# facebookresearch/habitat-lab

Measured on NVIDIA H100. Metric: DD-PPO learner frames/sec (ResNet18 RGB-D 256x256), higher is better.
Workload: dtype bf16

## Files before the change

### habitat-lab_b200/csrc/conv_halo.cu

```cuda
#include <cuda.h>
#include <stdlib.h>

#include "common.cuh"
#include "wgmma.cuh"

namespace hb200 {
void count_launch(int n);
using namespace wg;

constexpr int TH = 16, TW = 8;

__device__ __forceinline__ float warp_reduce16(float (&v)[16], int lane) {
  float a[8], b[4], c[2];
  const bool b4 = lane & 16, b3 = lane & 8, b2 = lane & 4, b1 = lane & 2;
#pragma unroll
  for (int i = 0; i < 8; ++i) a[i] = (b4 ? v[i + 8] : v[i]) + __shfl_xor_sync(0xffffffffu, b4 ? v[i] : v[i + 8], 16);
#pragma unroll
  for (int i = 0; i < 4; ++i) b[i] = (b3 ? a[i + 4] : a[i]) + __shfl_xor_sync(0xffffffffu, b3 ? a[i] : a[i + 4], 8);
#pragma unroll
  for (int i = 0; i < 2; ++i) c[i] = (b2 ? b[i + 2] : b[i]) + __shfl_xor_sync(0xffffffffu, b2 ? b[i] : b[i + 2], 4);
  float d = (b1 ? c[1] : c[0]) + __shfl_xor_sync(0xffffffffu, b1 ? c[0] : c[1], 2);
  d += __shfl_xor_sync(0xffffffffu, d, 1);
  return d;
}
// ... 340 lines not shown
      mbar_expect_tx(&dy_bar[st], (uint32_t)(DY_BYTES + (XMODE ? HROWS_LOAD * RP : 0)));
      tma_load_4d(sd, tmap_p, &dy_bar[st], 0, ow0, oh0, b);
      if (XMODE == 1) tma_load_5d(sd + DY_BYTES, tmap_xp, &dy_bar[st], 0, ow0 - PAD, 0, oh0 - PAD, b);
      if (XMODE == 2) tma_load_5d(sd + DY_BYTES, tmap_xp, &dy_bar[st], 0, ow0 - PAD, 0, 2 * (oh0 - PAD), b);
    }
  };
  const int first = blockIdx.x, stride = gridDim.x;
  const int my_n = first < a.ntiles ? (a.ntiles - first + stride - 1) / stride : 0;
  if (XMODE == 0 && my_n > 0) {
    fetch_x(first);
    commit_tile(first, 0);
  }
  cp_async_commit();
  fence_proxy_async_smem();
  __syncthreads();
  float acc_w[APC][N];
  auto mma_tile = [&](int it, uint32_t sd) {
    const uint32_t sh = sd + DY_BYTES;
    wgmma_fence();
#pragma unroll
    for (int l = 0; l < APC; ++l) {
      const int ai = grp * APC + l, s = ai / MT, mt = ai % MT;
#pragma unroll
      for (int ks = 0; ks < TH / 2; ++ks) {
        const uint64_t da = make_smem_desc(sh + 2 * ks * RP + s * 16 + mt * 16 * P, RP, P, kNoSwizzle);
        const uint64_t db = make_smem_desc(sd + ks * (16 * N * 2), 0, 8 * N * 2, N == 64 ? kSwizzle128B : kSwizzle64B);
        mma128<N, kBF16, 1, 1>(acc_w[l], da, 8 * P, db, (it > 0 || ks > 0) ? 1u : 0u);
      }
    }
    wgmma_commit();
    wgmma_wait<0>();
  };

  if (XMODE != 0) {
    if (tid == 0)
      for (int p = 0; p < NSW - 1 && p < my_n; ++p) commit_tile(first + p * stride, p);
    for (int it = 0; it < my_n; ++it) {
      const int nxt = it + NSW - 1;
      if (tid == 0 && nxt < my_n) commit_tile(first + nxt * stride, nxt % NSW);
      mbar_wait(&dy_bar[it % NSW], (it / NSW) & 1);
      mma_tile(it, sbase + (it % NSW) * STAGE);
    }
  } else {
    for (int it = 0; it < my_n; ++it) {
      const bool more = it + 1 < my_n;
      if (more) fetch_x(first + (it + 1) * stride);
      if (more) commit_tile(first + (it + 1) * stride, (it + 1) & 1);
      cp_async_commit();
      cp_async_wait<1>();
      fence_proxy_async_smem();
      __syncthreads();
      mbar_wait(&dy_bar[it & 1], (it >> 1) & 1);
      mma_tile(it, sbase + (it & 1) * STAGE);
    }
  }
  {
#pragma unroll
    for (int l = 0; l < APC; ++l) {
      if (my_n == 0) {
#pragma unroll
        for (int j = 0; j < N; ++j) acc_w[l][j] = 0.f;
      }
      acc_fence(acc_w[l]);
      const int ai = grp * APC + l, s = ai / MT, mt = ai % MT;
      const int blk = mt * 16 + (tid >> 3);
      const int r = blk / CJ, cj = blk % CJ;
      const bool ok = r < KH;
      const size_t row = (size_t)(r * KW + s) * C + cj * 8 + (tid & 7);
#pragma unroll
      for (int col0 = 0; col0 < N; col0 += 32) {
        float rr[32];
        acc_row32(acc_w[l], col0, stage_buf, rr);
        if (ok) {
          float* dst = a.dw + ((size_t)blockIdx.x * (KH * KW * C) + row) * N + col0;
#pragma unroll
          for (int j = 0; j < 32; j += 4) *reinterpret_cast<float4*>(dst + j) = make_float4(rr[j], rr[j + 1], rr[j + 2], rr[j + 3]);
        }
      }
    }
  }
}


constexpr int kSmallWgradStages = 3;
struct HaloWgradSmallArgs {
  const grad_t* x;
  const grad_t* dy;
  float* dw;
  int B, Ci, Co, ntiles;
};

template <int NS, int IMG>
__global__ void __launch_bounds__(128)
conv_halo_wgrad_small_kernel(const HaloWgradSmallArgs a, const __grid_constant__ CUtensorMap tmap_dy) {
  constexpr int CJ = 4, KH = 3, KW = 3, HWD = TW + KW - 1;
  constexpr int P = HWD * 16, RP = CJ * P;
  constexpr int IPT = TH / IMG;
  constexpr int RPI = IMG + 2;
  constexpr int HROWS_LOAD = IPT * RPI;
  constexpr int HROWS = (IPT - 1) * RPI + (IMG - 2) + 1 + 4;
  constexpr int HROWS_A = HROWS > HROWS_LOAD ? HROWS : HROWS_LOAD;
  constexpr int HALO_BYTES = (HROWS_A * RP + 1023) / 1024 * 1024;
  constexpr int NB = NS / 64;
  constexpr int DY_BYTES = NB * 128 * 128;
  constexpr int STAGE = HALO_BYTES + DY_BYTES;
  constexpr int NST = kSmallWgradStages;
  static_assert(NS <= 128, "one 128 x NS accumulator per CTA");
  extern __shared__ __align__(16) uint8_t smem_raw[];
  __shared__ __align__(8) uint64_t dy_bar[NST];
  __shared__ float stage_buf[kStageFloats];
  const uint32_t sbase = (smem_u32(smem_raw) + 1023u) & ~1023u;
  const int tid = threadIdx.x, warp = tid >> 5;
  const int nsl = a.Co / NS;
  const int s_tap = blockIdx.y % KW, slice = blockIdx.y / KW;
  const int c_off = (slice / nsl) * 32, n_off = (slice % nsl) * NS;
  const CUtensorMap* const tmap_p = &tmap_dy;

  if (tid == 0) {
#pragma unroll
    for (int i = 0; i < NST; ++i) mbar_init(&dy_bar[i], 1);
    mbar_fence_init();
  }
  for (int st = 0; st < NST; ++st)
    for (int v = tid; v < (HROWS_A - HROWS_LOAD) * RP / 16; v += 128) {
      const uint32_t addr = sbase + st * STAGE + HROWS_LOAD * RP + v * 16;
      asm volatile("st.shared.v4.b32 [%0], {%1,%1,%1,%1};" ::"r"(addr), "r"(0u) : "memory");
    }
  constexpr int XV = HROWS_LOAD * CJ * HWD, XPER = (XV + 95) / 96;
  uint4 xr[XPER];
  auto fetch_x = [&](int tile) {
    if (warp == 0) return;
    const int lt = tid - 32;
    const int b0 = tile * IPT;
#pragma unroll
    for (int i = 0; i < XPER; ++i) {
      const int v = lt + i * 96;
      uint4 r = make_uint4(0u, 0u, 0u, 0u);
      if (v < XV) {
        const int cj = v % CJ;
        const int t = v / CJ;
        const int hx = t % HWD, hy = t / HWD;
        const int j = hy / RPI, ih = hy - j * RPI - 1, iw = hx - 1;
        const int b = b0 + j;
        if (b < a.B && ih >= 0 && ih < IMG && iw >= 0 && iw < IMG)
          r = __ldg(reinterpret_cast<const uint4*>(a.x + ((((size_t)b * IMG + ih) * IMG + iw) * a.Ci + c_off + cj * 8)));
      }
      xr[i] = r;
    }
  };
  auto store_x = [&](int st) {
    if (warp == 0) return;
    const int lt = tid - 32;
    const uint32_t sh = sbase + st * STAGE;
#pragma unroll
    for (int i = 0; i < XPER; ++i) {
      const int v = lt + i * 96;
      if (v < XV) {
        const int cj = v % CJ;
        const int t = v / CJ;
        const int hx = t % HWD, hy = t / HWD;
        asm volatile("st.shared.v4.b32 [%0], {%1,%2,%3,%4};" ::"r"(sh + (uint32_t)(((hy * CJ + cj) * HWD + hx) * 16)),
                     "r"(xr[i].x), "r"(xr[i].y), "r"(xr[i].z), "r"(xr[i].w) : "memory");
      }
    }
  };
  auto load_dy = [&, tmap_p](int tile, int st) {
    const uint32_t sd = sbase + st * STAGE + HALO_BYTES;
    mbar_expect_tx(&dy_bar[st], (uint32_t)DY_BYTES);
#pragma unroll
    for (int nb = 0; nb < NB; ++nb)
      tma_load_4d(sd + (uint32_t)nb * (128 * 128), tmap_p, &dy_bar[st], n_off + nb * 64, 0, 0, tile * IPT);
  };
  const int first = blockIdx.x, stride = gridDim.x;
  const int my_n = first < a.ntiles ? (a.ntiles - first + stride - 1) / stride : 0;
#pragma unroll
  for (int i = 0; i < NST - 1; ++i) {
    if (i < my_n) {
      fetch_x(first + i * stride);
      store_x(i);
      if (tid == 0) load_dy(first + i * stride, i);
    }
  }
  fence_proxy_async_smem();
  __syncthreads();
  float acc_t[NS];

  for (int it = 0; it < my_n; ++it) {
    const int st = it % NST;
    const int nt = it + NST - 1;
    if (nt < my_n) fetch_x(first + nt * stride);
    fence_proxy_async_smem();
    __syncthreads();
    mbar_wait(&dy_bar[st], (it / NST) & 1);
    {
      const uint32_t sh = sbase + st * STAGE;
      const uint32_t sd = sh + HALO_BYTES;
      wgmma_fence();
#pragma unroll
      for (int ks = 0; ks < TH / 2; ++ks) {
        const int hb = ((2 * ks) / IMG) * RPI + (2 * ks) % IMG;
        const uint64_t da = make_smem_desc(sh + hb * RP + s_tap * 16, RP, P, kNoSwizzle);
        const uint64_t db = make_smem_desc(sd + ks * 2048, 128 * 128, 1024, kSwizzle128B);
        mma128<NS, kBF16, 1, 1>(acc_t, da, 8 * P, db, (it > 0 || ks > 0) ? 1u : 0u);
      }
      wgmma_commit();
      wgmma_wait<0>();
    }
    if (nt < my_n) {
      store_x(nt % NST);
      if (tid == 0) load_dy(first + nt * stride, nt % NST);
    }
  }
  {
    if (my_n == 0) {
#pragma unroll
      for (int j = 0; j < NS; ++j) acc_t[j] = 0.f;
    }
    acc_fence(acc_t);
    const int blk = tid >> 3;
    const int r = blk / CJ, cj = blk % CJ;
    const bool ok = r < KH;
    const size_t row = (size_t)(r * KW + s_tap) * a.Ci + c_off + cj * 8 + (tid & 7);
#pragma unroll
    for (int col0 = 0; col0 < NS; col0 += 32) {
      float rr[32];
      acc_row32(acc_t, col0, stage_buf, rr);
      if (ok) {
        float* dst = a.dw + ((size_t)blockIdx.x * 9 * a.Ci + row) * a.Co + n_off + col0;
#pragma unroll
        for (int j = 0; j < 32; j += 4) *reinterpret_cast<float4*>(dst + j) = make_float4(rr[j], rr[j + 1], rr[j + 2], rr[j + 3]);
      }
    }
  }
}

__global__ void pack_halo_weight_kernel(const float* __restrict__ w, __nv_bfloat16* __restrict__ img, int KH,
                                        int KW, int C, int N, int co, int ci_real, int mode) {
  const long long total = (long long)KH * KW * C * N;
  for (long long i = blockIdx.x * (long long)blockDim.x + threadIdx.x; i < total;
       i += (long long)gridDim.x * blockDim.x) {
    const int e = (int)(i & 7);
    long long t = i >> 3;
    const int n = (int)(t % N);
    t /= N;
    const int cj = (int)(t % (C / 8));
    const int tap = (int)(t / (C / 8));
    const int r = tap / KW, s = tap % KW, k = cj * 8 + e;
    float v = 0.f;
    if (mode == 0) {
      if (k < ci_real) v = w[(((size_t)n * ci_real + k) * KH + r) * KW + s];
    } else if (mode == 1) {
      if (n < ci_real) v = w[(((size_t)k * ci_real + n) * KH + (KH - 1 - r)) * KW + (KW - 1 - s)];
    } else {
      const int dy = k >> 3, dx = (k >> 2) & 1, c = k & 3;
      const int fr = 2 * r + dy - 1, fs = 2 * s + dx - 1;
      if (c < ci_real && fr >= 0 && fr < 7 && fs >= 0 && fs < 7) v = w[(((size_t)n * ci_real + c) * 7 + fr) * 7 + fs];
    }
    if (mode == 1) img[i] = __float2bfloat16(v);
    else reinterpret_cast<__half*>(img)[i] = __float2half_rn(v);
  }
}

__global__ void unpack_stem_wgrad_kernel(const float* __restrict__ acc, float* __restrict__ dw, int co, int ci_real) {
  const int total = co * ci_real * 49;
  for (int i = blockIdx.x * blockDim.x + threadIdx.x; i < total; i += gridDim.x * blockDim.x) {
    const int fs = i % 7, fr = (i / 7) % 7, c = (i / 49) % ci_real, o = i / (49 * ci_real);
    const int a = (fr + 1) >> 1, dy = (fr + 1) & 1, b = (fs + 1) >> 1, dx = (fs + 1) & 1;
    dw[i] = acc[((size_t)(a * 4 + b) * 16 + (dy * 2 + dx) * 4 + c) * co + o];
  }
}


template <int C, int N, int KH, int KW, int PAD, int MODE>
__global__ void __launch_bounds__(128)
conv_halo_tma_kernel(const HaloArgs a, const __grid_constant__ CUtensorMap tmap) {
  using Cfg = HaloCfg<C, N, KH, KW, PAD>;
  constexpr int CJ = Cfg::CJ, HH = Cfg::HH, HWD = Cfg::HWD;
  constexpr uint32_t SLAB = (uint32_t)((HH * HWD * 16 + 127) / 128 * 128);
  constexpr uint32_t STAGE = CJ * SLAB;
  constexpr int NB = (Cfg::W_BYTES + 2 * (int)STAGE > 110 * 1024) ? 1 : 2;
  extern __shared__ __align__(16) uint8_t smem_raw[];
  __shared__ __align__(8) uint64_t ld_bar[2];
  __shared__ float stage_buf[kStageFloats];
  const uint32_t sbase = (smem_u32(smem_raw) + 127u) & ~127u;
  const uint32_t s_w = sbase;
  const uint32_t s_halo0 = s_w + Cfg::W_BYTES;
  const int tid = threadIdx.x, lane = tid & 31;

  if (tid == 0) {
    mbar_init(&ld_bar[0], 1);
    mbar_init(&ld_bar[1], 1);
    mbar_fence_init();
  }
  {
    const uint4* src = reinterpret_cast<const uint4*>(a.wimg);
    for (int v = tid; v < Cfg::W_BYTES / 16; v += 128) cp_async16(s_w + (uint32_t)v * 16, src + v, true);
  }
  cp_async_commit();
  const int tiles_x = a.W / TW, tiles_y = a.H / TH;
  const int tiles_per_img = tiles_x * tiles_y;
  auto tile_coords = [&](int tile, int& b, int& oh0, int& ow0) {
    b = tile / tiles_per_img;
    const int r = tile - b * tiles_per_img;
    oh0 = (r / tiles_x) * TH;
    ow0 = (r % tiles_x) * TW;
  };
  const CUtensorMap* const tmap_p = &tmap;
  auto issue_halo = [&, tmap_p](int tile, int stage) {
    int b, oh0, ow0;
    tile_coords(tile, b, oh0, ow0);
    mbar_expect_tx(&ld_bar[stage], (uint32_t)(CJ * HH * HWD * 16));
#pragma unroll
    for (int j = 0; j < CJ; ++j)
// ... 269 lines not shown
    const int py = t >> 3, px = t & 7;
    float* const stage_buf = stage_bufs + wgi * kStageFloats;
    float acc_t[N];
    for (int it = wgi; it < my_n; it += 2) {
      const int st = it % NS;
      const int tile = first + it * stride;
      const int b = tile / tiles_per_img, r = tile - b * tiles_per_img;
      const int oh0 = (r / tiles_x) * TH, ow0 = (r % tiles_x) * TW;
      mbar_wait(&full_bar[st], (it / NS) & 1);
      const uint32_t sh = s_halo0 + (uint32_t)st * STAGE;
      wgmma_fence();
      uint32_t accum = 0;
#pragma unroll
      for (int r = 0; r < KH; ++r)
#pragma unroll
        for (int s = 0; s < KW; ++s)
#pragma unroll
          for (int kk = 0; kk < C / 16; ++kk) {
            const uint64_t da = SW ? make_smem_desc(sh + s * COPY + r * ATOM + kk * 32, 16, ATOM, (Layout)kSw)
                                   : make_smem_desc(sh + 2 * kk * SLAB + r * (HWD * 16) + s * 16, SLAB, HWD * 16, kNoSwizzle);
            const uint64_t db = make_smem_desc(s_w + (r * KW + s) * (C * N * 2) + 2 * kk * (N * 16), N * 16, 128, kNoSwizzle);
            mma128<N, kT>(acc_t, da, SW ? 8 * ATOM : 8 * HWD * 16, db, accum);
            accum = 1;
          }
      wgmma_commit();
      wgmma_wait<0>();
      acc_fence(acc_t);
      if (t == 0) mbar_arrive(&empty_bar[st]);
      const size_t pix = ((size_t)b * a.H + oh0 + py) * a.W + ow0 + px;
#pragma unroll
      for (int col0 = 0; col0 < N; col0 += 32) {
        float acc_[32];
        acc_row32(acc_t, col0, stage_buf, acc_, 1 + wgi);
        if (MODE == 0 && a.stats != nullptr)
          halo_gn_stats_chunk(acc_, lane, N / a.gn_groups, a.stats + (size_t)b * a.gn_groups * 2, col0);
        const size_t o = pix * N + col0;
        if (MODE == 1 && a.addend != nullptr) {
          const uint4* ad = reinterpret_cast<const uint4*>(a.addend + o);
#pragma unroll
          for (int v = 0; v < 4; ++v) {
            float f[8];
            unpack8(ad[v], f);
#pragma unroll
            for (int e2 = 0; e2 < 8; ++e2) acc_[v * 8 + e2] += f[e2];
          }
        }
        uint4* dst = reinterpret_cast<uint4*>(a.y + o);
#pragma unroll
        for (int v = 0; v < 4; ++v) {
          uint4 u;
          if (MODE == 0) {
            u.x = pack_f16x2(acc_[v * 8 + 0], acc_[v * 8 + 1]);
            u.y = pack_f16x2(acc_[v * 8 + 2], acc_[v * 8 + 3]);
            u.z = pack_f16x2(acc_[v * 8 + 4], acc_[v * 8 + 5]);
            u.w = pack_f16x2(acc_[v * 8 + 6], acc_[v * 8 + 7]);
          } else {
            u.x = pack_bf16x2(acc_[v * 8 + 0], acc_[v * 8 + 1]);
            u.y = pack_bf16x2(acc_[v * 8 + 2], acc_[v * 8 + 3]);
            u.z = pack_bf16x2(acc_[v * 8 + 4], acc_[v * 8 + 5]);
            u.w = pack_bf16x2(acc_[v * 8 + 6], acc_[v * 8 + 7]);
          }
          dst[v] = u;
        }
      }
    }
  }
}

typedef CUresult (*EncodeTiledFn)(CUtensorMap*, CUtensorMapDataType, cuuint32_t, void*, const cuuint64_t*,
                                  const cuuint64_t*, const cuuint32_t*, const cuuint32_t*, CUtensorMapInterleave,
                                  CUtensorMapSwizzle, CUtensorMapL2promotion, CUtensorMapFloatOOBfill);
static EncodeTiledFn halo_encode_fn() {
  static EncodeTiledFn fn = nullptr;
  if (fn) return fn;
  void* p = nullptr;
  cudaDriverEntryPointQueryResult q;
  if (cudaGetDriverEntryPoint("cuTensorMapEncodeTiled", &p, cudaEnableDefault, &q) != cudaSuccess ||
      q != cudaDriverEntryPointSuccess)
    return nullptr;
  fn = (EncodeTiledFn)p;
  return fn;
}

static int blocks_per_sm(const void* kern, size_t smem, int* cache) {
  if (*cache > 0) return *cache;
  cudaFuncAttributes fa;
  if (cudaFuncGetAttributes(&fa, kern) != cudaSuccess) return 1;
  const int regs = fa.numRegs > 0 ? fa.numRegs : 128;
  int by_regs = 65536 / (((regs + 7) / 8 * 8) * 128);
  int by_smem = (int)((227 * 1024) / (smem + fa.sharedSizeBytes + 1024));
  int n = by_regs < by_smem ? by_regs : by_smem;
  if (n > 16) n = 16;
  if (n < 1) n = 1;
  *cache = n;
  return n;
}

template <int C, int N, int KH, int KW, int PAD, int MODE>
static int launch_halo(const HaloArgs& a, cudaStream_t st) {
  using Cfg = HaloCfg<C, N, KH, KW, PAD>;
  const size_t smem = Cfg::W_BYTES + Cfg::NBUF * Cfg::HALO_BYTES + 256;
  auto kern = conv_halo_kernel<C, N, KH, KW, PAD, MODE>;
  static int cache = 0;
  if (cache == 0) HB_CUDA(cudaFuncSetAttribute(kern, cudaFuncAttributeMaxDynamicSharedMemorySize, (int)smem));
  const int per_sm = blocks_per_sm((const void*)kern, smem, &cache);
  int grid = kNumSMs * per_sm;
  if (grid > a.ntiles) grid = a.ntiles;
  kern<<<grid, 128, smem, st>>>(a);
  HB_LAUNCH_OK();
  count_launch(1);
  return HB200_OK;
}

template <int C, int N, int KH, int KW, int PAD, int MODE>
static int launch_halo_tma(const HaloArgs& a, cudaStream_t st) {
  using Cfg = HaloCfg<C, N, KH, KW, PAD>;
  EncodeTiledFn enc = halo_encode_fn();
  if (!enc) {
    set_last_error("conv_halo (TMA): cuTensorMapEncodeTiled is not available from this driver");
    return HB200_ERR_UNSUPPORTED;
  }
  CUtensorMap tmap;
  const cuuint64_t dims[4] = {(cuuint64_t)C, (cuuint64_t)a.W, (cuuint64_t)a.H, (cuuint64_t)a.B};
  const cuuint64_t strides[3] = {(cuuint64_t)C * 2, (cuuint64_t)a.W * C * 2, (cuuint64_t)a.H * a.W * C * 2};
  const cuuint32_t box[4] = {8u, (cuuint32_t)Cfg::HWD, (cuuint32_t)Cfg::HH, 1u};
  const cuuint32_t estr[4] = {1u, 1u, 1u, 1u};
  const CUresult r = enc(&tmap, CU_TENSOR_MAP_DATA_TYPE_BFLOAT16, 4, (void*)a.x, dims, strides, box, estr,
                         CU_TENSOR_MAP_INTERLEAVE_NONE, CU_TENSOR_MAP_SWIZZLE_NONE, CU_TENSOR_MAP_L2_PROMOTION_L2_128B,
                         CU_TENSOR_MAP_FLOAT_OOB_FILL_NONE);
  if (r != CUDA_SUCCESS) {
    set_last_error("conv_halo (TMA): cuTensorMapEncodeTiled failed (%d)", (int)r);
    return HB200_ERR_CUDA;
  }
  constexpr size_t slab = (size_t)((Cfg::HH * Cfg::HWD * 16 + 127) / 128 * 128);
  constexpr int nstage = (Cfg::W_BYTES + 2 * (int)(Cfg::CJ * slab) > 110 * 1024) ? 1 : 2;
  const size_t smem = Cfg::W_BYTES + nstage * Cfg::CJ * slab + 256;
  auto kern = conv_halo_tma_kernel<C, N, KH, KW, PAD, MODE>;
  static int cache = 0;
  if (cache == 0) HB_CUDA(cudaFuncSetAttribute(kern, cudaFuncAttributeMaxDynamicSharedMemorySize, (int)smem));
  const int per_sm = blocks_per_sm((const void*)kern, smem, &cache);
  int grid = kNumSMs * per_sm;
  if (grid > a.ntiles) grid = a.ntiles;
  kern<<<grid, 128, smem, st>>>(a, tmap);
  HB_LAUNCH_OK();
  count_launch(1);
  return HB200_OK;
}

template <int C, int N, int KH, int KW, int PAD, int MODE, int NS, bool SW = false>
static int launch_halo_ws(const HaloArgs& a, cudaStream_t st) {
  using Cfg = HaloCfg<C, N, KH, KW, PAD>;
  EncodeTiledFn enc = halo_encode_fn();
  if (!enc) {
    set_last_error("conv_halo (TMA): cuTensorMapEncodeTiled is not available from this driver");
    return HB200_ERR_UNSUPPORTED;
  }
  CUtensorMap tmap;
  const cuuint64_t dims[4] = {(cuuint64_t)C, (cuuint64_t)a.W, (cuuint64_t)a.H, (cuuint64_t)a.B};
  const cuuint64_t strides[3] = {(cuuint64_t)C * 2, (cuuint64_t)a.W * C * 2, (cuuint64_t)a.H * a.W * C * 2};
  const cuuint32_t box_slab[4] = {8u, (cuuint32_t)Cfg::HWD, (cuuint32_t)Cfg::HH, 1u};
  const cuuint32_t box_rows[4] = {(cuuint32_t)C, (cuuint32_t)TW, (cuuint32_t)Cfg::HH, 1u};
  const cuuint32_t* box = SW ? box_rows : box_slab;
  const cuuint32_t estr[4] = {1u, 1u, 1u, 1u};
  const CUresult r = enc(&tmap, CU_TENSOR_MAP_DATA_TYPE_BFLOAT16, 4, (void*)a.x, dims, strides, box, estr,
                         CU_TENSOR_MAP_INTERLEAVE_NONE,
                         !SW ? CU_TENSOR_MAP_SWIZZLE_NONE : (C == 64 ? CU_TENSOR_MAP_SWIZZLE_128B : CU_TENSOR_MAP_SWIZZLE_64B),
                         CU_TENSOR_MAP_L2_PROMOTION_L2_128B, CU_TENSOR_MAP_FLOAT_OOB_FILL_NONE);
  if (r != CUDA_SUCCESS) {
    set_last_error("conv_halo (TMA): cuTensorMapEncodeTiled failed (%d)", (int)r);
    return HB200_ERR_CUDA;
  }
  constexpr size_t slab = (size_t)((Cfg::HH * Cfg::HWD * 16 + 127) / 128 * 128);
// ... 37 lines not shown
                         CU_TENSOR_MAP_L2_PROMOTION_L2_128B, CU_TENSOR_MAP_FLOAT_OOB_FILL_NONE);
  if (r != CUDA_SUCCESS) {
    set_last_error("conv_halo (swizzled TMA): cuTensorMapEncodeTiled failed (%d)", (int)r);
    return HB200_ERR_CUDA;
  }
  constexpr size_t stage = (size_t)3 * Cfg::HH * 8 * C * 2;
  constexpr int nstage = (Cfg::W_BYTES + 2 * (int)stage > 200 * 1024) ? 1 : 2;
  const size_t smem = Cfg::W_BYTES + nstage * stage + 1024;
  auto kern = conv_halo_sw_kernel<C, N, MODE>;
  static int cache = 0;
  if (cache == 0) HB_CUDA(cudaFuncSetAttribute(kern, cudaFuncAttributeMaxDynamicSharedMemorySize, (int)smem));
  const int per_sm = blocks_per_sm((const void*)kern, smem, &cache);
  int grid = kNumSMs * per_sm;
  if (grid > a.ntiles) grid = a.ntiles;
  kern<<<grid, 128, smem, st>>>(a, tmap);
  HB_LAUNCH_OK();
  count_launch(1);
  return HB200_OK;
}

template <int C, int N, int KH, int KW, int PAD, int XMODE = 0>
static int launch_halo_wgrad(const HaloWgradArgs& a, cudaStream_t st) {
  constexpr int CJ = C / 8, HWD = TW + KW - 1, P = HWD * 16, RP = CJ * P;
  constexpr int MT = (KH * CJ + 15) / 16, RMAX = (MT * 16 + CJ - 1) / CJ, HROWS = TH - 1 + RMAX;
  constexpr int STAGE = (128 * N * 2 + HROWS * RP + 1023) / 1024 * 1024;
  constexpr int NSW = halo_wgrad_stages(XMODE, C, STAGE);
  const size_t smem = NSW * (size_t)STAGE + 1024 + 64;
  EncodeTiledFn enc = halo_encode_fn();
  if (!enc) {
    set_last_error("conv_halo_wgrad: cuTensorMapEncodeTiled is not available from this driver");
    return HB200_ERR_UNSUPPORTED;
  }
  CUtensorMap tmap;
  const cuuint64_t dims[4] = {(cuuint64_t)N, (cuuint64_t)a.W, (cuuint64_t)a.H, (cuuint64_t)a.B};
  const cuuint64_t strides[3] = {(cuuint64_t)N * 2, (cuuint64_t)a.W * N * 2, (cuuint64_t)a.H * a.W * N * 2};
  const cuuint32_t box[4] = {(cuuint32_t)N, (cuuint32_t)TW, (cuuint32_t)TH, 1u};
  const cuuint32_t estr[4] = {1u, 1u, 1u, 1u};
  const CUresult r = enc(&tmap, CU_TENSOR_MAP_DATA_TYPE_BFLOAT16, 4, (void*)a.dy, dims, strides, box, estr,
                         CU_TENSOR_MAP_INTERLEAVE_NONE, N == 64 ? CU_TENSOR_MAP_SWIZZLE_128B : CU_TENSOR_MAP_SWIZZLE_64B,
                         CU_TENSOR_MAP_L2_PROMOTION_L2_128B, CU_TENSOR_MAP_FLOAT_OOB_FILL_NONE);
  if (r != CUDA_SUCCESS) {
    set_last_error("conv_halo_wgrad: cuTensorMapEncodeTiled failed (%d)", (int)r);
    return HB200_ERR_CUDA;
  }
  CUtensorMap tmap_x = tmap;
  if (XMODE != 0) {
    const int cx = XMODE == 2 ? C / 4 : C, hx = XMODE == 2 ? 2 * a.H : a.H, wx = XMODE == 2 ? 2 * a.W : a.W;
    const int chunks_per_row = XMODE == 2 ? CJ / 2 : CJ, col_bytes = (XMODE == 2 ? 2 : 1) * cx * 2;
    const cuuint64_t xd[5] = {8u, (cuuint64_t)a.W, (cuuint64_t)chunks_per_row, (cuuint64_t)hx, (cuuint64_t)a.B};
    const cuuint64_t xs[4] = {(cuuint64_t)col_bytes, 16u, (cuuint64_t)wx * cx * 2, (cuuint64_t)hx * wx * cx * 2};
    constexpr int HROWS_LOAD = TH + KH - 1;
    const cuuint32_t xb[5] = {8u, (cuuint32_t)HWD, (cuuint32_t)chunks_per_row,
                              (cuuint32_t)(XMODE == 2 ? 2 * HROWS_LOAD : HROWS_LOAD), 1u};
    const cuuint32_t xe[5] = {1u, 1u, 1u, 1u, 1u};
    const CUresult rx = enc(&tmap_x, CU_TENSOR_MAP_DATA_TYPE_BFLOAT16, 5, (void*)a.x, xd, xs, xb, xe,
                            CU_TENSOR_MAP_INTERLEAVE_NONE, CU_TENSOR_MAP_SWIZZLE_NONE, CU_TENSOR_MAP_L2_PROMOTION_L2_128B,
                            CU_TENSOR_MAP_FLOAT_OOB_FILL_NONE);
    if (rx != CUDA_SUCCESS) {
      set_last_error("conv_halo_wgrad: cuTensorMapEncodeTiled (x halo) failed (%d)", (int)rx);
      return HB200_ERR_CUDA;
    }
  }
  auto kern = conv_halo_wgrad_kernel<C, N, KH, KW, PAD, XMODE>;
  static int cache = 0;
  if (cache == 0) HB_CUDA(cudaFuncSetAttribute(kern, cudaFuncAttributeMaxDynamicSharedMemorySize, (int)smem));
  constexpr int nacc = KW * MT, ngrp = nacc * N <= 128 ? 1 : nacc / (128 / N);
  const int per_sm = blocks_per_sm((const void*)kern, smem, &cache);
  int grid = kNumSMs * per_sm / ngrp;
  if (grid < 1) grid = 1;
  if (grid > a.ntiles) grid = a.ntiles;
  const long long count = (long long)KH * KW * C * N;
  float* parts = nullptr;
  int* tickets = nullptr;
  int rc = stream_workspace(st, (size_t)(grid + (grid < kReduceChunks ? grid : kReduceChunks)) * count, 0, &parts, &tickets);
  if (rc) return rc;
  HaloWgradArgs ap = a;
  ap.dw = parts;
  kern<<<dim3(grid, ngrp), 128, smem, st>>>(ap, tmap, tmap_x);
  HB_LAUNCH_OK();
  count_launch(1);
  return reduce_partials(parts, grid, count, count, a.dw, parts + (size_t)grid * count, st);
}

template <int NS, int IMG>
static int launch_halo_wgrad_small(const HaloWgradSmallArgs& a, cudaStream_t st) {
  constexpr int RP = 4 * (TW + 2) * 16, IPT = TH / IMG, RPI = IMG + 2;
  constexpr int HROWS_LOAD = IPT * RPI, HROWS = (IPT - 1) * RPI + (IMG - 2) + 1 + 4;
  constexpr int HROWS_A = HROWS > HROWS_LOAD ? HROWS : HROWS_LOAD;
  constexpr int HALO_BYTES = (HROWS_A * RP + 1023) / 1024 * 1024;
  const size_t smem = kSmallWgradStages * (size_t)(HALO_BYTES + (NS / 64) * 128 * 128) + 1024 + 64;
  EncodeTiledFn enc = halo_encode_fn();
  if (!enc) {
    set_last_error("conv_halo_wgrad (small images): cuTensorMapEncodeTiled is not available from this driver");
    return HB200_ERR_UNSUPPORTED;
  }
  CUtensorMap tmap;
  const cuuint64_t dims[4] = {(cuuint64_t)a.Co, (cuuint64_t)IMG, (cuuint64_t)IMG, (cuuint64_t)a.B};
  const cuuint64_t strides[3] = {(cuuint64_t)a.Co * 2, (cuuint64_t)IMG * a.Co * 2, (cuuint64_t)IMG * IMG * a.Co * 2};
  const cuuint32_t box[4] = {64u, 8u, (cuuint32_t)IMG, (cuuint32_t)IPT};
  const cuuint32_t estr[4] = {1u, 1u, 1u, 1u};
  const CUresult r = enc(&tmap, CU_TENSOR_MAP_DATA_TYPE_BFLOAT16, 4, (void*)a.dy, dims, strides, box, estr,
                         CU_TENSOR_MAP_INTERLEAVE_NONE, CU_TENSOR_MAP_SWIZZLE_128B, CU_TENSOR_MAP_L2_PROMOTION_L2_128B,
                         CU_TENSOR_MAP_FLOAT_OOB_FILL_NONE);
  if (r != CUDA_SUCCESS) {
    set_last_error("conv_halo_wgrad (small images): cuTensorMapEncodeTiled failed (%d)", (int)r);
    return HB200_ERR_CUDA;
  }
  auto kern = conv_halo_wgrad_small_kernel<NS, IMG>;
  static bool attr = false;
  if (!attr) {
    HB_CUDA(cudaFuncSetAttribute(kern, cudaFuncAttributeMaxDynamicSharedMemorySize, (int)smem));
    attr = true;
  }
  const int slices = (a.Ci / 32) * (a.Co / NS) * 3;
  int workers = 2 * kNumSMs / slices;
  if (workers < 1) workers = 1;
  if (workers > a.ntiles) workers = a.ntiles;
  const long long count = 9LL * a.Ci * a.Co;
  float* parts = nullptr;
  int* tickets = nullptr;
  int rc = stream_workspace(st, (size_t)(workers + (workers < kReduceChunks ? workers : kReduceChunks)) * count, 0, &parts,
                            &tickets);
  if (rc) return rc;
  HaloWgradSmallArgs ap = a;
  ap.dw = parts;
  kern<<<dim3(workers, slices), 128, smem, st>>>(ap, tmap);
  HB_LAUNCH_OK();
  count_launch(1);
  return reduce_partials(parts, workers, count, count, a.dw, parts + (size_t)workers * count, st);
}
}

using namespace hb200;

static int g_halo_tma = getenv("HB200_NO_HALO_TMA") == nullptr ? 1 : 0;
static int g_wgrad_xtma = getenv("HB200_WGRAD_XTMA") ? atoi(getenv("HB200_WGRAD_XTMA")) : 1;
extern "C" int hb200_set_halo_tma(int enable) {
  g_halo_tma = enable;
  return HB200_OK;
}
extern "C" int hb200_get_halo_tma(void) { return g_halo_tma; }

extern "C" int hb200_conv_halo_supported(int c, int n, int k, int h, int w) {
  if (h % TH || w % TW) return 0;
  if (k == 3) return (c == 32 && n == 32) || (c == 64 && n == 64);
  if (k == 4) return c == 16 && n == 32;
  return 0;
}

extern "C" int hb200_conv_halo_wgrad_supported(int c, int n, int k, int h, int w) {
  if (hb200_conv_halo_supported(c, n, k, h, w)) return 1;
  return k == 3 && c % 32 == 0 && n % 128 == 0 && h == w && (h == 8 || h == 4);
}

extern "C" int hb200_pack_halo_weight(const float* w_oihw, hb200_bf16* img, int co, int ci_real, int c, int n,
                                      int k, int mode, hb200_stream_t stream) {
  HB_CHECK_ARG(w_oihw && img && mode >= 0 && mode <= 2, "pack_halo_weight: bad args");
  const long long total = (long long)k * k * c * n;
  pack_halo_weight_kernel<<<(int)min((total + 255) / 256, (long long)kNumSMs * 4), 256, 0, (cudaStream_t)stream>>>(
      w_oihw, (__nv_bfloat16*)img, k, k, c, n, co, ci_real, mode);
  HB_LAUNCH_OK();
  count_launch(1);
  return HB200_OK;
}

extern "C" int hb200_unpack_stem_wgrad(const float* dw_acc, float* dw_oihw, int co, int ci_real,
                                       hb200_stream_t stream) {
  HB_CHECK_ARG(dw_acc && dw_oihw && ci_real <= 4, "unpack_stem_wgrad: bad args");
  unpack_stem_wgrad_kernel<<<cdiv(co * ci_real * 49, 256), 256, 0, (cudaStream_t)stream>>>(dw_acc, dw_oihw, co, ci_real);
  HB_LAUNCH_OK();
  count_launch(1);
  return HB200_OK;
}

extern "C" int hb200_conv_halo(const hb200_bf16* x, const hb200_bf16* wimg, hb200_bf16* y, const hb200_bf16* addend,
                               double* gn_stats, int gn_groups, int batch, int h, int w, int c, int n, int k,
                               int mode, hb200_stream_t stream) {
  HB_CHECK_ARG(x && wimg && y, "conv_halo: null pointer");
  HB_CHECK_ARG(hb200_conv_halo_supported(c, n, k, h, w), "conv_halo: unsupported shape C=%d N=%d k=%d %dx%d", c, n, k, h, w);
  if (gn_stats) HB_CHECK_ARG(gn_groups > 0 && n % gn_groups == 0 && n / gn_groups >= 2, "conv_halo: bad GroupNorm groups");
  HaloArgs a;
  a.x = (const __nv_bfloat16*)x; a.wimg = (const __nv_bfloat16*)wimg; a.y = (__nv_bfloat16*)y;
  a.addend = (const __nv_bfloat16*)addend; a.stats = gn_stats;
  a.B = batch; a.H = h; a.W = w; a.gn_groups = gn_groups > 0 ? gn_groups : 1;
  a.ntiles = batch * (h / TH) * (w / TW);
  cudaStream_t st = (cudaStream_t)stream;
  const bool use_tma = g_halo_tma != 0;
  if (g_halo_tma == 1 && k == 3 && c == 64)
    return mode == 0 ? launch_halo_ws<64, 64, 3, 3, 1, 0, 2, true>(a, st) : launch_halo_ws<64, 64, 3, 3, 1, 1, 2, true>(a, st);
  if (g_halo_tma == 1 && k == 3 && c == 32)
    return mode == 0 ? launch_halo_ws<32, 32, 3, 3, 1, 0, 6, true>(a, st) : launch_halo_ws<32, 32, 3, 3, 1, 1, 6, true>(a, st);
  if (g_halo_tma == 1 && k == 4 && mode == 0) return launch_halo_ws<16, 32, 4, 4, 2, 0, 6>(a, st);
  if (g_halo_tma == 6 && k == 3 && c == 32)
    return mode == 0 ? launch_halo_ws<32, 32, 3, 3, 1, 0, 2, true>(a, st) : launch_halo_ws<32, 32, 3, 3, 1, 1, 2, true>(a, st);
  if (g_halo_tma == 4 && k == 3 && c == 32)
    return mode == 0 ? launch_halo_ws<32, 32, 3, 3, 1, 0, 3, true>(a, st) : launch_halo_ws<32, 32, 3, 3, 1, 1, 3, true>(a, st);
  if (g_halo_tma == 4 && k == 3 && c == 64)
    return mode == 0 ? launch_halo_ws<64, 64, 3, 3, 1, 0, 2, true>(a, st) : launch_halo_ws<64, 64, 3, 3, 1, 1, 2, true>(a, st);
  if (g_halo_tma == 3 && k == 3 && c == 32)
    return mode == 0 ? launch_halo_ws<32, 32, 3, 3, 1, 0, 4>(a, st) : launch_halo_ws<32, 32, 3, 3, 1, 1, 4>(a, st);
  if (g_halo_tma == 3 && k == 3 && c == 64)
    return mode == 0 ? launch_halo_ws<64, 64, 3, 3, 1, 0, 5>(a, st) : launch_halo_ws<64, 64, 3, 3, 1, 1, 5>(a, st);
  if (g_halo_tma == 3 && k == 4 && mode == 0) return launch_halo_ws<16, 32, 4, 4, 2, 0, 6>(a, st);
  if (g_halo_tma == 2 && k == 3 && c == 32)
    return mode == 0 ? launch_halo_sw<32, 32, 0>(a, st) : launch_halo_sw<32, 32, 1>(a, st);
  if (g_halo_tma == 2 && k == 3 && c == 64)
    return mode == 0 ? launch_halo_sw<64, 64, 0>(a, st) : launch_halo_sw<64, 64, 1>(a, st);
  if (use_tma && k == 3 && c == 32)
    return mode == 0 ? launch_halo_tma<32, 32, 3, 3, 1, 0>(a, st) : launch_halo_tma<32, 32, 3, 3, 1, 1>(a, st);
  if (use_tma && k == 4 && mode == 0) return launch_halo_tma<16, 32, 4, 4, 2, 0>(a, st);
  if (use_tma && k == 3 && c == 64)
    return mode == 0 ? launch_halo_tma<64, 64, 3, 3, 1, 0>(a, st) : launch_halo_tma<64, 64, 3, 3, 1, 1>(a, st);
  if (k == 3 && c == 32) return mode == 0 ? launch_halo<32, 32, 3, 3, 1, 0>(a, st) : launch_halo<32, 32, 3, 3, 1, 1>(a, st);
  if (k == 3 && c == 64) return mode == 0 ? launch_halo<64, 64, 3, 3, 1, 0>(a, st) : launch_halo<64, 64, 3, 3, 1, 1>(a, st);
  HB_CHECK_ARG(mode == 0, "conv_halo: the stem has no data gradient");
  return launch_halo<16, 32, 4, 4, 2, 0>(a, st);
}

__global__ void unpack_s2_wgrad_kernel(const float* __restrict__ acc, float* __restrict__ dw, int co, int ci) {
  const int total = co * ci * 9;
  for (int i = blockIdx.x * blockDim.x + threadIdx.x; i < total; i += gridDim.x * blockDim.x) {
    const int s = i % 3, r = (i / 3) % 3, c = (i / 9) % ci, o = i / (9 * ci);
    const int ky = r == 0 ? 0 : 1, dy = r == 0 ? 1 : r - 1, kx = s == 0 ? 0 : 1, dx = s == 0 ? 1 : s - 1;
    dw[i] = acc[((size_t)((ky * 2 + kx) * 4 + dy * 2 + dx) * ci + c) * co + o];
  }
}

extern "C" int hb200_conv_s2_wgrad_supported(int c, int n, int h, int w) {
  return c == 32 && n == 64 && h % (2 * TH) == 0 && w % (2 * TW) == 0;
}
extern "C" int hb200_conv_s2_wgrad(const hb200_bf16* x, const hb200_bf16* dy, float* dw_acc, int batch, int h, int w,
                                   int c, int n, hb200_stream_t stream) {
  HB_CHECK_ARG(x && dy && dw_acc && batch > 0, "conv_s2_wgrad: null pointer");
  HB_CHECK_ARG(hb200_conv_s2_wgrad_supported(c, n, h, w), "conv_s2_wgrad: unsupported shape C=%d N=%d %dx%d", c, n, h, w);
  HaloWgradArgs a;
  a.x = (const __nv_bfloat16*)x; a.dy = (const __nv_bfloat16*)dy; a.dw = dw_acc;
  a.B = batch; a.H = h / 2; a.W = w / 2;
  a.ntiles = batch * (a.H / TH) * (a.W / TW);
  return launch_halo_wgrad<128, 64, 2, 2, 1, 2>(a, (cudaStream_t)stream);
}
extern "C" int hb200_unpack_s2_wgrad(const float* dw_acc, float* dw_oihw, int co, int ci, hb200_stream_t stream) {
  HB_CHECK_ARG(dw_acc && dw_oihw && co > 0 && ci > 0, "unpack_s2_wgrad: bad args");
  unpack_s2_wgrad_kernel<<<cdiv(co * ci * 9, 256), 256, 0, (cudaStream_t)stream>>>(dw_acc, dw_oihw, co, ci);
  HB_LAUNCH_OK();
  count_launch(1);
  return HB200_OK;
}

extern "C" int hb200_conv_halo_wgrad(const hb200_bf16* x, const hb200_bf16* dy, float* dw_acc, int batch, int h,
                                     int w, int c, int n, int k, hb200_stream_t stream) {
  HB_CHECK_ARG(x && dy && dw_acc, "conv_halo_wgrad: null pointer");
  HB_CHECK_ARG(hb200_conv_halo_wgrad_supported(c, n, k, h, w), "conv_halo_wgrad: unsupported shape C=%d N=%d k=%d %dx%d", c, n, k, h, w);
  if (!hb200_conv_halo_supported(c, n, k, h, w)) {
    HaloWgradSmallArgs s;
    s.x = (const grad_t*)x; s.dy = (const grad_t*)dy; s.dw = dw_acc;
    s.B = batch; s.Ci = c; s.Co = n;
    const int ipt = TH / h;
    s.ntiles = (batch + ipt - 1) / ipt;
    return h == 8 ? launch_halo_wgrad_small<128, 8>(s, (cudaStream_t)stream) : launch_halo_wgrad_small<128, 4>(s, (cudaStream_t)stream);
  }
  HaloWgradArgs a;
  a.x = (const __nv_bfloat16*)x; a.dy = (const __nv_bfloat16*)dy; a.dw = dw_acc;
  a.B = batch; a.H = h; a.W = w;
  a.ntiles = batch * (h / TH) * (w / TW);
  cudaStream_t st = (cudaStream_t)stream;
  if (g_wgrad_xtma) {
    if (k == 3 && c == 32) return launch_halo_wgrad<32, 32, 3, 3, 1, 1>(a, st);
    if (k == 3 && c == 64) return launch_halo_wgrad<64, 64, 3, 3, 1, 1>(a, st);
    return launch_halo_wgrad<16, 32, 4, 4, 2, 1>(a, st);
  }
  if (k == 3 && c == 32) return launch_halo_wgrad<32, 32, 3, 3, 1>(a, st);
  if (k == 3 && c == 64) return launch_halo_wgrad<64, 64, 3, 3, 1>(a, st);
  return launch_halo_wgrad<16, 32, 4, 4, 2>(a, st);
}
extern "C" int hb200_set_wgrad_xtma(int on) { g_wgrad_xtma = on ? 1 : 0; return HB200_OK; }
extern "C" int hb200_get_wgrad_xtma(void) { return g_wgrad_xtma; }
```

Before: 57400.

## Warp-specialize small-image halo wgrad with TMA producer and deep mbarrier pipeline

Replaces the 128-thread small-image weight-gradient kernel with a 416-thread warp-specialized kernel. One producer warpgroup loads both dy and the x halo through TMA (a new 5D tensor map), feeding up to 8 stages guarded by full/empty mbarriers. Three consumer warpgroups each handle one kernel row and use 64-channel input blocks. This removes register-staged x loads and per-iteration __syncthreads, and keeps one wgmma group in flight. The grid is now sized from measured occupancy. The cost is large shared memory per CTA and fewer CTAs per SM.

New measurement: 59880, median of 6. 1.04x the previous value.

```diff
diff --git a/habitat-lab_b200/csrc/conv_halo.cu b/habitat-lab_b200/csrc/conv_halo.cu
--- a/habitat-lab_b200/csrc/conv_halo.cu
+++ b/habitat-lab_b200/csrc/conv_halo.cu
@@ -446,153 +446,109 @@
 }
 
 
-constexpr int kSmallWgradStages = 3;
-struct HaloWgradSmallArgs {
-  const grad_t* x;
-  const grad_t* dy;
+constexpr int kWgradSmallThreads = 416;
+constexpr int kWgradSmallCols = 128;
+struct WgradSmallArgs {
   float* dw;
-  int B, Ci, Co, ntiles;
+  int Ci, Co, ntiles;
 };
 
-template <int NS, int IMG>
-__global__ void __launch_bounds__(128)
-conv_halo_wgrad_small_kernel(const HaloWgradSmallArgs a, const __grid_constant__ CUtensorMap tmap_dy) {
-  constexpr int CJ = 4, KH = 3, KW = 3, HWD = TW + KW - 1;
-  constexpr int P = HWD * 16, RP = CJ * P;
-  constexpr int IPT = TH / IMG;
-  constexpr int RPI = IMG + 2;
-  constexpr int HROWS_LOAD = IPT * RPI;
-  constexpr int HROWS = (IPT - 1) * RPI + (IMG - 2) + 1 + 4;
-  constexpr int HROWS_A = HROWS > HROWS_LOAD ? HROWS : HROWS_LOAD;
-  constexpr int HALO_BYTES = (HROWS_A * RP + 1023) / 1024 * 1024;
-  constexpr int NB = NS / 64;
-  constexpr int DY_BYTES = NB * 128 * 128;
-  constexpr int STAGE = HALO_BYTES + DY_BYTES;
-  constexpr int NST = kSmallWgradStages;
-  static_assert(NS <= 128, "one 128 x NS accumulator per CTA");
+template <int IMG>
+struct WgradSmallCfg {
+  static constexpr int NIMG = TH / IMG;
+  static constexpr int ROWB = IMG * 16;
+  static constexpr int CHUNK = NIMG * (IMG + 2) * ROWB;
+  static constexpr int XB = 8 * CHUNK;
+  static constexpr int DYBLK = TH * TW * 128;
+  static constexpr int DYB = kWgradSmallCols / 64 * DYBLK;
+  static constexpr int GAP = 1024;
+  static constexpr int STAGE = DYB + XB + GAP;
+  static constexpr int NS_FIT = (227 * 1024 - 1024 - 256) / STAGE;
+  static constexpr int NS = NS_FIT < 8 ? NS_FIT : 8;
+  static constexpr size_t SMEM = (size_t)NS * STAGE + 1024;
+  static_assert(XB % 1024 == 0 && NS >= 3, "stage layout");
+};
+
+template <int IMG>
+__global__ void __launch_bounds__(kWgradSmallThreads, 1)
+conv_wgrad_small_ws_kernel(const WgradSmallArgs a, const __grid_constant__ CUtensorMap tmap_dy,
+                           const __grid_constant__ CUtensorMap tmap_x) {
+  using Cfg = WgradSmallCfg<IMG>;
+  constexpr int NS = Cfg::NS, STAGE = Cfg::STAGE, NCO = kWgradSmallCols;
   extern __shared__ __align__(16) uint8_t smem_raw[];
-  __shared__ __align__(8) uint64_t dy_bar[NST];
-  __shared__ float stage_buf[kStageFloats];
+  __shared__ __align__(8) uint64_t full_bar[NS], empty_bar[NS];
   const uint32_t sbase = (smem_u32(smem_raw) + 1023u) & ~1023u;
-  const int tid = threadIdx.x, warp = tid >> 5;
-  const int nsl = a.Co / NS;
-  const int s_tap = blockIdx.y % KW, slice = blockIdx.y / KW;
-  const int c_off = (slice / nsl) * 32, n_off = (slice % nsl) * NS;
-  const CUtensorMap* const tmap_p = &tmap_dy;
-
+  const int tid = threadIdx.x, wg_id = tid >> 7, t = tid & 127;
+  const int nci = (a.Ci + 63) / 64;
+  const int s_tap = blockIdx.y % 3, cb = (blockIdx.y / 3) % nci, nb = blockIdx.y / (3 * nci);
   if (tid == 0) {
 #pragma unroll
-    for (int i = 0; i < NST; ++i) mbar_init(&dy_bar[i], 1);
+    for (int i = 0; i < NS; ++i) {
+      mbar_init(&full_bar[i], 1);
+      mbar_init(&empty_bar[i], 3);
+    }
     mbar_fence_init();
   }
-  for (int st = 0; st < NST; ++st)
-    for (int v = tid; v < (HROWS_A - HROWS_LOAD) * RP / 16; v += 128) {
-      const uint32_t addr = sbase + st * STAGE + HROWS_LOAD * RP + v * 16;
-      asm volatile("st.shared.v4.b32 [%0], {%1,%1,%1,%1};" ::"r"(addr), "r"(0u) : "memory");
-    }
-  constexpr int XV = HROWS_LOAD * CJ * HWD, XPER = (XV + 95) / 96;
-  uint4 xr[XPER];
-  auto fetch_x = [&](int tile) {
-    if (warp == 0) return;
-    const int lt = tid - 32;
-    const int b0 = tile * IPT;
-#pragma unroll
-    for (int i = 0; i < XPER; ++i) {
-      const int v = lt + i * 96;
-      uint4 r = make_uint4(0u, 0u, 0u, 0u);
-      if (v < XV) {
-        const int cj = v % CJ;
-        const int t = v / CJ;
-        const int hx = t % HWD, hy = t / HWD;
-        const int j = hy / RPI, ih = hy - j * RPI - 1, iw = hx - 1;
-        const int b = b0 + j;
-        if (b < a.B && ih >= 0 && ih < IMG && iw >= 0 && iw < IMG)
-          r = __ldg(reinterpret_cast<const uint4*>(a.x + ((((size_t)b * IMG + ih) * IMG + iw) * a.Ci + c_off + cj * 8)));
-      }
-      xr[i] = r;
-    }
-  };
-  auto store_x = [&](int st) {
-    if (warp == 0) return;
-    const int lt = tid - 32;
-    const uint32_t sh = sbase + st * STAGE;
-#pragma unroll
-    for (int i = 0; i < XPER; ++i) {
-      const int v = lt + i * 96;
-      if (v < XV) {
-        const int cj = v % CJ;
-        const int t = v / CJ;
-        const int hx = t % HWD, hy = t / HWD;
-        asm volatile("st.shared.v4.b32 [%0], {%1,%2,%3,%4};" ::"r"(sh + (uint32_t)(((hy * CJ + cj) * HWD + hx) * 16)),
-                     "r"(xr[i].x), "r"(xr[i].y), "r"(xr[i].z), "r"(xr[i].w) : "memory");
-      }
-    }
-  };
-  auto load_dy = [&, tmap_p](int tile, int st) {
-    const uint32_t sd = sbase + st * STAGE + HALO_BYTES;
-    mbar_expect_tx(&dy_bar[st], (uint32_t)DY_BYTES);
-#pragma unroll
-    for (int nb = 0; nb < NB; ++nb)
-      tma_load_4d(sd + (uint32_t)nb * (128 * 128), tmap_p, &dy_bar[st], n_off + nb * 64, 0, 0, tile * IPT);
-  };
+  if (tid < NS * 8)
+    asm volatile("st.shared.v4.b32 [%0], {%1,%1,%1,%1};" ::"r"(sbase + (tid / 8) * STAGE + Cfg::DYB + Cfg::XB + (tid % 8) * 16),
+                 "r"(0u) : "memory");
+  fence_proxy_async_smem();
+  __syncthreads();
   const int first = blockIdx.x, stride = gridDim.x;
   const int my_n = first < a.ntiles ? (a.ntiles - first + stride - 1) / stride : 0;
-#pragma unroll
-  for (int i = 0; i < NST - 1; ++i) {
-    if (i < my_n) {
-      fetch_x(first + i * stride);
-      store_x(i);
-      if (tid == 0) load_dy(first + i * stride, i);
-    }
-  }
-  fence_proxy_async_smem();
-  __syncthreads();
-  float acc_t[NS];
-
-  for (int it = 0; it < my_n; ++it) {
-    const int st = it % NST;
-    const int nt = it + NST - 1;
-    if (nt < my_n) fetch_x(first + nt * stride);
-    fence_proxy_async_smem();
-    __syncthreads();
-    mbar_wait(&dy_bar[st], (it / NST) & 1);
-    {
-      const uint32_t sh = sbase + st * STAGE;
-      const uint32_t sd = sh + HALO_BYTES;
+
+  if (wg_id == 3) {
+    if (t == 0) {
+      const CUtensorMap* const pd = &tmap_dy;
+      const CUtensorMap* const px = &tmap_x;
+      for (int it = 0; it < my_n; ++it) {
+        const int st = it % NS;
+        if (it >= NS) mbar_wait(&empty_bar[st], ((it / NS) - 1) & 1);
+        const int b0 = (first + it * stride) * Cfg::NIMG;
+        const uint32_t sd = sbase + (uint32_t)st * STAGE;
+        mbar_expect_tx(&full_bar[st], (uint32_t)(Cfg::DYB + Cfg::XB));
+#pragma unroll
+        for (int j = 0; j < NCO / 64; ++j)
+          tma_load_4d(sd + (uint32_t)j * Cfg::DYBLK, pd, &full_bar[st], nb * NCO + j * 64, 0, 0, b0);
+        tma_load_5d(sd + Cfg::DYB, px, &full_bar[st], 0, s_tap - 1, -1, b0, cb * 8);
+      }
+    }
+  } else {
+    const int r = wg_id;
+    float acc[NCO / 2];
+    for (int it = 0; it < my_n; ++it) {
+      const int st = it % NS;
+      mbar_wait(&full_bar[st], (it / NS) & 1);
+      const uint32_t sd = sbase + (uint32_t)st * STAGE, sx = sd + Cfg::DYB;
       wgmma_fence();
 #pragma unroll
-      for (int ks = 0; ks < TH / 2; ++ks) {
-        const int hb = ((2 * ks) / IMG) * RPI + (2 * ks) % IMG;
-        const uint64_t da = make_smem_desc(sh + hb * RP + s_tap * 16, RP, P, kNoSwizzle);
-        const uint64_t db = make_smem_desc(sd + ks * 2048, 128 * 128, 1024, kSwizzle128B);
-        mma128<NS, kBF16, 1, 1>(acc_t, da, 8 * P, db, (it > 0 || ks > 0) ? 1u : 0u);
+      for (int k = 0; k < TH / 2; ++k) {
+        const int j = (2 * k) / IMG, oh0 = (2 * k) % IMG;
+        const uint64_t da = make_smem_desc(sx + (uint32_t)((j * (IMG + 2) + oh0 + r) * Cfg::ROWB), Cfg::ROWB, Cfg::CHUNK,
+                                           kNoSwizzle);
+        const uint64_t db = make_smem_desc(sd + (uint32_t)k * 2048, Cfg::DYBLK, 1024, kSwizzle128B);
+        Wgmma<NCO, kBF16>::template mma<1, 1>(acc, da, db, (it > 0 || k > 0) ? 1u : 0u);
       }
       wgmma_commit();
-      wgmma_wait<0>();
-    }
-    if (nt < my_n) {
-      store_x(nt % NST);
-      if (tid == 0) load_dy(first + nt * stride, nt % NST);
-    }
-  }
-  {
+      wgmma_wait<1>();
+      if (it > 0 && t == 0) mbar_arrive(&empty_bar[(it - 1) % NS]);
+    }
+    wgmma_wait<0>();
     if (my_n == 0) {
 #pragma unroll
-      for (int j = 0; j < NS; ++j) acc_t[j] = 0.f;
-    }
-    acc_fence(acc_t);
-    const int blk = tid >> 3;
-    const int r = blk / CJ, cj = blk % CJ;
-    const bool ok = r < KH;
-    const size_t row = (size_t)(r * KW + s_tap) * a.Ci + c_off + cj * 8 + (tid & 7);
-#pragma unroll
-    for (int col0 = 0; col0 < NS; col0 += 32) {
-      float rr[32];
-      acc_row32(acc_t, col0, stage_buf, rr);
-      if (ok) {
-        float* dst = a.dw + ((size_t)blockIdx.x * 9 * a.Ci + row) * a.Co + n_off + col0;
-#pragma unroll
-        for (int j = 0; j < 32; j += 4) *reinterpret_cast<float4*>(dst + j) = make_float4(rr[j], rr[j + 1], rr[j + 2], rr[j + 3]);
+      for (int i = 0; i < NCO / 2; ++i) acc[i] = 0.f;
+    }
+    acc_fence(acc);
+    const int w = t >> 5, l = t & 31;
+    const int ci = cb * 64 + 16 * w + (l >> 2);
+    float* const dst = a.dw + ((size_t)blockIdx.x * 9 * a.Ci + (size_t)(r * 3 + s_tap) * a.Ci + ci) * a.Co +
+                       nb * NCO + 2 * (l & 3);
+#pragma unroll
+    for (int h = 0; h < 2; ++h) {
+      if (ci + 8 * h < a.Ci) {
+#pragma unroll
+        for (int i = 0; i < NCO / 8; ++i)
+          *reinterpret_cast<float2*>(dst + (size_t)(8 * h) * a.Co + 8 * i) = make_float2(acc[4 * i + 2 * h], acc[4 * i + 2 * h + 1]);
       }
     }
   }
@@ -1028,12 +984,12 @@
   return fn;
 }
 
-static int blocks_per_sm(const void* kern, size_t smem, int* cache) {
+static int blocks_per_sm(const void* kern, size_t smem, int* cache, int threads = 128) {
   if (*cache > 0) return *cache;
   cudaFuncAttributes fa;
   if (cudaFuncGetAttributes(&fa, kern) != cudaSuccess) return 1;
   const int regs = fa.numRegs > 0 ? fa.numRegs : 128;
-  int by_regs = 65536 / (((regs + 7) / 8 * 8) * 128);
+  int by_regs = 65536 / (((regs + 7) / 8 * 8) * threads);
   int by_smem = (int)((227 * 1024) / (smem + fa.sharedSizeBytes + 1024));
   int n = by_regs < by_smem ? by_regs : by_smem;
   if (n > 16) n = 16;
@@ -1237,52 +1193,56 @@
   return reduce_partials(parts, grid, count, count, a.dw, parts + (size_t)grid * count, st);
 }
 
-template <int NS, int IMG>
-static int launch_halo_wgrad_small(const HaloWgradSmallArgs& a, cudaStream_t st) {
-  constexpr int RP = 4 * (TW + 2) * 16, IPT = TH / IMG, RPI = IMG + 2;
-  constexpr int HROWS_LOAD = IPT * RPI, HROWS = (IPT - 1) * RPI + (IMG - 2) + 1 + 4;
-  constexpr int HROWS_A = HROWS > HROWS_LOAD ? HROWS : HROWS_LOAD;
-  constexpr int HALO_BYTES = (HROWS_A * RP + 1023) / 1024 * 1024;
-  const size_t smem = kSmallWgradStages * (size_t)(HALO_BYTES + (NS / 64) * 128 * 128) + 1024 + 64;
+template <int IMG>
+static int launch_wgrad_small(const grad_t* x, const grad_t* dy, float* dw, int B, int Ci, int Co, cudaStream_t st) {
+  using Cfg = WgradSmallCfg<IMG>;
   EncodeTiledFn enc = halo_encode_fn();
   if (!enc) {
     set_last_error("conv_halo_wgrad (small images): cuTensorMapEncodeTiled is not available from this driver");
     return HB200_ERR_UNSUPPORTED;
   }
-  CUtensorMap tmap;
-  const cuuint64_t dims[4] = {(cuuint64_t)a.Co, (cuuint64_t)IMG, (cuuint64_t)IMG, (cuuint64_t)a.B};
-  const cuuint64_t strides[3] = {(cuuint64_t)a.Co * 2, (cuuint64_t)IMG * a.Co * 2, (cuuint64_t)IMG * IMG * a.Co * 2};
-  const cuuint32_t box[4] = {64u, 8u, (cuuint32_t)IMG, (cuuint32_t)IPT};
-  const cuuint32_t estr[4] = {1u, 1u, 1u, 1u};
-  const CUresult r = enc(&tmap, CU_TENSOR_MAP_DATA_TYPE_BFLOAT16, 4, (void*)a.dy, dims, strides, box, estr,
-                         CU_TENSOR_MAP_INTERLEAVE_NONE, CU_TENSOR_MAP_SWIZZLE_128B, CU_TENSOR_MAP_L2_PROMOTION_L2_128B,
-                         CU_TENSOR_MAP_FLOAT_OOB_FILL_NONE);
+  CUtensorMap tmap_dy, tmap_x;
+  const cuuint64_t dims[4] = {(cuuint64_t)Co, (cuuint64_t)IMG, (cuuint64_t)IMG, (cuuint64_t)B};
+  const cuuint64_t strides[3] = {(cuuint64_t)Co * 2, (cuuint64_t)IMG * Co * 2, (cuuint64_t)IMG * IMG * Co * 2};
+  const cuuint32_t box[4] = {64u, (cuuint32_t)TW, (cuuint32_t)IMG, (cuuint32_t)Cfg::NIMG};
+  const cuuint32_t estr[5] = {1u, 1u, 1u, 1u, 1u};
+  CUresult r = enc(&tmap_dy, CU_TENSOR_MAP_DATA_TYPE_BFLOAT16, 4, (void*)dy, dims, strides, box, estr,
+                   CU_TENSOR_MAP_INTERLEAVE_NONE, CU_TENSOR_MAP_SWIZZLE_128B, CU_TENSOR_MAP_L2_PROMOTION_L2_128B,
+                   CU_TENSOR_MAP_FLOAT_OOB_FILL_NONE);
   if (r != CUDA_SUCCESS) {
-    set_last_error("conv_halo_wgrad (small images): cuTensorMapEncodeTiled failed (%d)", (int)r);
+    set_last_error("conv_halo_wgrad (small images): cuTensorMapEncodeTiled (dy) failed (%d)", (int)r);
     return HB200_ERR_CUDA;
   }
-  auto kern = conv_halo_wgrad_small_kernel<NS, IMG>;
-  static bool attr = false;
-  if (!attr) {
-    HB_CUDA(cudaFuncSetAttribute(kern, cudaFuncAttributeMaxDynamicSharedMemorySize, (int)smem));
-    attr = true;
-  }
-  const int slices = (a.Ci / 32) * (a.Co / NS) * 3;
-  int workers = 2 * kNumSMs / slices;
+  const cuuint64_t xd[5] = {8u, (cuuint64_t)IMG, (cuuint64_t)IMG, (cuuint64_t)B, (cuuint64_t)(Ci / 8)};
+  const cuuint64_t xs[4] = {(cuuint64_t)Ci * 2, (cuuint64_t)IMG * Ci * 2, (cuuint64_t)IMG * IMG * Ci * 2, 16u};
+  const cuuint32_t xb[5] = {8u, (cuuint32_t)IMG, (cuuint32_t)(IMG + 2), (cuuint32_t)Cfg::NIMG, 8u};
+  r = enc(&tmap_x, CU_TENSOR_MAP_DATA_TYPE_BFLOAT16, 5, (void*)x, xd, xs, xb, estr, CU_TENSOR_MAP_INTERLEAVE_NONE,
+          CU_TENSOR_MAP_SWIZZLE_NONE, CU_TENSOR_MAP_L2_PROMOTION_L2_128B, CU_TENSOR_MAP_FLOAT_OOB_FILL_NONE);
+  if (r != CUDA_SUCCESS) {
+    set_last_error("conv_halo_wgrad (small images): cuTensorMapEncodeTiled (x) failed (%d)", (int)r);
+    return HB200_ERR_CUDA;
+  }
+  auto kern = conv_wgrad_small_ws_kernel<IMG>;
+  static int cache = 0;
+  if (cache == 0) HB_CUDA(cudaFuncSetAttribute(kern, cudaFuncAttributeMaxDynamicSharedMemorySize, (int)Cfg::SMEM));
+  const int per_sm = blocks_per_sm((const void*)kern, Cfg::SMEM, &cache, kWgradSmallThreads);
+  const int ntiles = (B + Cfg::NIMG - 1) / Cfg::NIMG;
+  const int slices = (Ci + 63) / 64 * 3 * (Co / kWgradSmallCols);
+  int workers = kNumSMs * per_sm / slices;
   if (workers < 1) workers = 1;
-  if (workers > a.ntiles) workers = a.ntiles;
-  const long long count = 9LL * a.Ci * a.Co;
+  if (workers > ntiles) workers = ntiles;
+  const long long count = 9LL * Ci * Co;
   float* parts = nullptr;
   int* tickets = nullptr;
   int rc = stream_workspace(st, (size_t)(workers + (workers < kReduceChunks ? workers : kReduceChunks)) * count, 0, &parts,
                             &tickets);
   if (rc) return rc;
-  HaloWgradSmallArgs ap = a;
-  ap.dw = parts;
-  kern<<<dim3(workers, slices), 128, smem, st>>>(ap, tmap);
+  WgradSmallArgs a;
+  a.dw = parts; a.Ci = Ci; a.Co = Co; a.ntiles = ntiles;
+  kern<<<dim3(workers, slices), kWgradSmallThreads, Cfg::SMEM, st>>>(a, tmap_dy, tmap_x);
   HB_LAUNCH_OK();
   count_launch(1);
-  return reduce_partials(parts, workers, count, count, a.dw, parts + (size_t)workers * count, st);
+  return reduce_partials(parts, workers, count, count, dw, parts + (size_t)workers * count, st);
 }
 }
 
@@ -1407,12 +1367,10 @@
   HB_CHECK_ARG(x && dy && dw_acc, "conv_halo_wgrad: null pointer");
   HB_CHECK_ARG(hb200_conv_halo_wgrad_supported(c, n, k, h, w), "conv_halo_wgrad: unsupported shape C=%d N=%d k=%d %dx%d", c, n, k, h, w);
   if (!hb200_conv_halo_supported(c, n, k, h, w)) {
-    HaloWgradSmallArgs s;
-    s.x = (const grad_t*)x; s.dy = (const grad_t*)dy; s.dw = dw_acc;
-    s.B = batch; s.Ci = c; s.Co = n;
-    const int ipt = TH / h;
-    s.ntiles = (batch + ipt - 1) / ipt;
-    return h == 8 ? launch_halo_wgrad_small<128, 8>(s, (cudaStream_t)stream) : launch_halo_wgrad_small<128, 4>(s, (cudaStream_t)stream);
+    const grad_t* xg = (const grad_t*)x;
+    const grad_t* dyg = (const grad_t*)dy;
+    cudaStream_t st = (cudaStream_t)stream;
+    return h == 8 ? launch_wgrad_small<8>(xg, dyg, dw_acc, batch, c, n, st) : launch_wgrad_small<4>(xg, dyg, dw_acc, batch, c, n, st);
   }
   HaloWgradArgs a;
   a.x = (const __nv_bfloat16*)x; a.dy = (const __nv_bfloat16*)dy; a.dw = dw_acc;
```
